# refresh-bio/vclust

Hardware: AMD Instinct MI355X
Metric: genome pairs/sec through prefilter+align (ani.tsv) (higher is better)
Workload: dtype u64

## Files before the change

vclust_amd/build.py:

```python
import os
import pathlib
import shutil
import subprocess
import sys

PKG_DIR = pathlib.Path(__file__).resolve().parent
ROOT = PKG_DIR.parent
CSRC = PKG_DIR / 'csrc'
LIB_PATH = PKG_DIR / 'libvclust_gpu.so'
ORACLE_DIR = ROOT / 'oracle'

SOURCES = ['vg_core.cpp', 'vg_genomes.cpp', 'vg_inflate.cpp', 'vg_io.cpp', 'vg_api.cpp', 'vg_synth.cpp', 'vg_prefilter.hip', 'vg_align.hip', 'vg_dist.hip', 'vg_cluster.hip', 'vg_dedup.hip']


def _hipcc() -> str:
    for cand in (os.environ.get('HIPCC'), shutil.which('hipcc'), '/opt/rocm/bin/hipcc'):
        if cand and pathlib.Path(cand).exists():
            return cand
    raise RuntimeError('hipcc not found (needs ROCm)')


def _stale(target: pathlib.Path, deps) -> bool:
    if not target.exists():
        return True
    t = target.stat().st_mtime
    return any(pathlib.Path(d).stat().st_mtime > t for d in deps)


def build_lib(force: bool = False, verbose: bool = False) -> pathlib.Path:
    srcs = [CSRC / s for s in SOURCES]
    deps = srcs + [CSRC / 'vg_common.h', CSRC / 'vg_window.h', ROOT / 'include' / 'vclust_gpu.h']
    if not force and not _stale(LIB_PATH, deps):
        return LIB_PATH
    obj_dir = PKG_DIR / '_obj'
    obj_dir.mkdir(exist_ok=True)
    hipcc = _hipcc()
    flags = ['--offload-arch=gfx950', '-O3', '-std=c++17', '-fPIC', '-Wall', '-Wno-unused-function',
             '-Wno-unused-result', f'-I{ROOT / "include"}']
    if os.environ.get('VG_LINES') == '1':
        flags.append('-gline-tables-only')
    if os.environ.get('VG_DEV') == '1':
        flags.append('-DVG_DEV_KERNELS')
    objs = []
    procs = []
    for s in srcs:
        o = obj_dir / (s.name + '.o')
        objs.append(o)
        if force or _stale(o, [s, CSRC / 'vg_common.h', CSRC / 'vg_window.h', ROOT / 'include' / 'vclust_gpu.h']):
            cmd = [hipcc, *flags, '-x', 'hip', '-c', str(s), '-o', str(o)]
            if verbose:
                print(' '.join(cmd), file=sys.stderr)
            procs.append((s, subprocess.Popen(cmd, stdout=subprocess.PIPE, stderr=subprocess.STDOUT, text=True)))
    for s, p in procs:
        out, _ = p.communicate()
        if p.returncode != 0:
            raise RuntimeError(f'hipcc failed on {s.name}:\n{out}')
        if verbose and out.strip():
            print(out, file=sys.stderr)
    cmd = [hipcc, '--offload-arch=gfx950', '-shared', '-fPIC', '-o', str(LIB_PATH), *map(str, objs), '-lz', '-lpthread', '-ldl']
    r = subprocess.run(cmd, stdout=subprocess.PIPE, stderr=subprocess.STDOUT, text=True)
    if r.returncode != 0:
        raise RuntimeError(f'link failed:\n{r.stdout}')
    return LIB_PATH


def build_oracle(verbose: bool = False) -> pathlib.Path:
    r = subprocess.run(['make', '-C', str(ORACLE_DIR)], stdout=subprocess.PIPE, stderr=subprocess.STDOUT, text=True)
    if r.returncode != 0:
        raise RuntimeError(f'oracle build failed:\n{r.stdout}')
    if verbose:
        print(r.stdout, file=sys.stderr)
    return ORACLE_DIR / '_build' / 'liboracle.so'


if __name__ == '__main__':
    force = '--force' in sys.argv
    print(build_lib(force=force, verbose=True))
    print(build_oracle(verbose=False))
```

vclust_amd/csrc/vg_align.hip:

```cpp
#include "vg_common.h"
#include "vg_window.h"
#include <rocprim/rocprim.hpp>
#include <algorithm>
#include <numeric>
#include <cstring>
#include <memory>
#include <mutex>
#include <optional>

namespace {

constexpr int RR_PAD = 128;

struct ref_desc {
    int64_t rr_w;
    int64_t mask_w;
    int64_t stab;
    int64_t sent;
    int32_t L;
    int32_t n_rr;
    int32_t genome;
    int32_t has_n;
    int32_t pos_bits;
    int32_t tag_bits;
// ... 371 lines not shown
#pragma unroll
                for (int u = 0; u < 4; ++u) {
                    const int p0 = pb + u * 4 * (int)blockDim.x;
                    if (p0 >= n4) continue;
                    const uint32_t sh = (uint32_t)(p0 & 31);
                    const uint32_t XL = __builtin_amdgcn_alignbit(w4[u].z, w4[u].x, sh), XH = __builtin_amdgcn_alignbit(w4[u].w, w4[u].y, sh);
                    const uint32_t XM = __builtin_amdgcn_alignbit(m1[u], m0[u], sh);
                    uint32_t out[4];
#pragma unroll
                    for (int j = 0; j < 4; ++j) {
                        const int p = p0 + j;
                        uint32_t bt = 0xffffffffu;
                        if (p + w <= rd.n_rr && ((XM >> j) & ((1u << w) - 1u)) == 0) {
                            const uint32_t xl = XL >> j, xh = XH >> j;
                            bt = bucket_of(xl, xh, msl) | (tag_of(xl, xh, msl, rd.tag_bits) << 18);
                            atomicAdd(&tab[(bt & 0x3ffffu) >> (big ? tsh : 0)], 1u);
                        }
                        out[j] = bt;
                    }
                    *reinterpret_cast<uint4*>(&scratch[p0]) = make_uint4(out[0], out[1], out[2], out[3]);
                }
            }
            __threadfence_block();
            __syncthreads();
            if (!big) {
                const uint32_t total = lds_scan_exclusive_waves(tab, n_cnt, part);
                const int nb = n_cnt;
                int w_lo = 0;
                while (w_lo < nb) {
                    const uint32_t base = tab[w_lo];
                    if (threadIdx.x == 0) s_whi = w_lo + 1;
                    lds_sync();
                    int best = w_lo + 1;
                    for (int b2 = w_lo + threadIdx.x; b2 < nb; b2 += blockDim.x) {
                        const uint32_t e2 = (b2 + 1 < nb) ? tab[b2 + 1] : total;
                        if (e2 - base <= (uint32_t)LDS_STAGE) best = b2 + 1; else break;
                    }
                    atomicMax(&s_whi, best);
                    lds_sync();
                    const int w_hi = s_whi;
                    const uint32_t e_lo = (w_lo + 1 < nb) ? tab[w_lo + 1] : total;
                    const bool direct = (e_lo - base > (uint32_t)LDS_STAGE);
                    lds_sync();
                    for (int pb = 4 * threadIdx.x; pb < n4; pb += 16 * blockDim.x) {
                        uint4 v[4];
#pragma unroll
                        for (int u = 0; u < 4; ++u) {
                            const int p0 = pb + u * 4 * (int)blockDim.x;
                            v[u] = (p0 < n4) ? *reinterpret_cast<const uint4*>(&scratch[p0]) : make_uint4(~0u, ~0u, ~0u, ~0u);
                        }
#pragma unroll
                        for (int u = 0; u < 4; ++u) {
                            const int p0 = pb + u * 4 * (int)blockDim.x;
                            const uint32_t bts[4] = { v[u].x, v[u].y, v[u].z, v[u].w };
#pragma unroll
                            for (int j = 0; j < 4; ++j) {
                                const uint32_t bt = bts[j];
                                const int b2 = (int)(bt & 0x3ffffu);
                                if (bt == 0xffffffffu || b2 < w_lo || b2 >= w_hi) continue;
                                const uint32_t ent = (uint32_t)(p0 + j) | ((bt >> 18) << rd.pos_bits);
                                const uint32_t slot = atomicAdd(&tab[b2], 1u);
                                if (direct) gent[slot] = ent; else stage[slot - base] = ent;
                            }
                        }
                    }
                    lds_sync();
                    if (!direct) {
                        const uint32_t cnt = tab[w_hi - 1] - base;
                        for (uint32_t i = threadIdx.x; i < cnt; i += blockDim.x) gent[base + i] = stage[i];
                    }
                    lds_sync();
                    w_lo = w_hi;
                }
                for (int i = threadIdx.x; i < nb; i += blockDim.x) gtab[i] = tab[i];
                lds_sync();
                continue;
            }
            const int n_bins = n_cnt;
            const uint32_t total = lds_scan_exclusive_waves(tab, n_bins, part);
            for (int i = threadIdx.x; i <= n_bins; i += blockDim.x) { s_bstart[i] = i < n_bins ? tab[i] : total; }
            lds_sync();
            for (int pb = 4 * threadIdx.x; pb < n4; pb += 16 * blockDim.x) {
                uint4 v[4];
#pragma unroll
                for (int u = 0; u < 4; ++u) {
                    const int p0 = pb + u * 4 * (int)blockDim.x;
                    v[u] = (p0 < n4) ? *reinterpret_cast<const uint4*>(&scratch[p0]) : make_uint4(~0u, ~0u, ~0u, ~0u);
                }
#pragma unroll
                for (int u = 0; u < 4; ++u) {
                    const int p0 = pb + u * 4 * (int)blockDim.x;
                    const uint32_t bts[4] = { v[u].x, v[u].y, v[u].z, v[u].w };
#pragma unroll
                    for (int j = 0; j < 4; ++j) {
                        if (bts[j] == 0xffffffffu) continue;
                        const uint32_t slot = atomicAdd(&tab[(bts[j] & 0x3ffffu) >> tsh], 1u);
                        binned[slot] = make_uint2(bts[j], (uint32_t)(p0 + j));
                    }
                }
            }
            __threadfence_block();
            __syncthreads();
            const int per_bin = 1 << tsh;
            int w_lo = 0;
            while (w_lo < n_bins) {
                if (threadIdx.x == 0) {
                    int hi = w_lo + 1;
                    while (hi < n_bins && s_bstart[hi + 1] - s_bstart[w_lo] <= (uint32_t)LDS_STAGE && (hi + 1 - w_lo) * per_bin <= LDS_TAB) ++hi;
                    s_whi = hi;
                }
                lds_sync();
                const int w_hi = s_whi;
                const uint32_t base = s_bstart[w_lo], cnt = s_bstart[w_hi] - base;
                const int nbw = (w_hi - w_lo) * per_bin; const uint32_t b_lo = (uint32_t)w_lo << tsh;
                const bool direct = cnt > (uint32_t)LDS_STAGE;
                for (int i = threadIdx.x; i < nbw; i += blockDim.x) tab[i] = 0;
                lds_sync();
                for (uint32_t i0 = threadIdx.x; i0 < cnt; i0 += 4 * blockDim.x) {
                    uint32_t bx[4];
#pragma unroll
                    for (int u = 0; u < 4; ++u) { const uint32_t i = i0 + u * blockDim.x; bx[u] = i < cnt ? binned[base + i].x : 0xffffffffu; }
#pragma unroll
                    for (int u = 0; u < 4; ++u) if (i0 + u * blockDim.x < cnt) atomicAdd(&tab[(bx[u] & 0x3ffffu) - b_lo], 1u);
                }
                lds_sync();
                lds_scan_exclusive_waves(tab, nbw, part);
                for (uint32_t i0 = threadIdx.x; i0 < cnt; i0 += 4 * blockDim.x) {
                    uint2 e4[4];
#pragma unroll
                    for (int u = 0; u < 4; ++u) { const uint32_t i = i0 + u * blockDim.x; e4[u] = i < cnt ? binned[base + i] : make_uint2(0u, 0u); }
#pragma unroll
                    for (int u = 0; u < 4; ++u) {
                        if (i0 + u * blockDim.x >= cnt) continue;
                        const uint2 e = e4[u];
                        const uint32_t ent = e.y | ((e.x >> 18) << rd.pos_bits);
                        const uint32_t slot = atomicAdd(&tab[(e.x & 0x3ffffu) - b_lo], 1u);
                        if (direct) gent[base + slot] = ent; else stage[slot] = ent;
                    }
                }
                lds_sync();
                if (!direct) for (uint32_t i = threadIdx.x; i < cnt; i += blockDim.x) gent[base + i] = stage[i];
                for (int i = threadIdx.x; i < nbw; i += blockDim.x) gtab[b_lo + i] = base + tab[i];
                lds_sync();
                w_lo = w_hi;
            }
        }
    }
}

constexpr int REG_IT = 24;
constexpr int REG_MAX_RR = 4 * 1024 * REG_IT - 256;
constexpr int REG_RR_WORDS = REG_MAX_RR / 16 + 32;
constexpr int REG_MK_WORDS = REG_MAX_RR / 32 + 16;
constexpr int REG_GEN_WORDS = 12288;
constexpr int REG_LDS_WORDS = LDS_TAB + REG_GEN_WORDS + REG_RR_WORDS + REG_MK_WORDS;
constexpr int REG_STAGE = REG_LDS_WORDS / 1024 * 1024;
constexpr int REG_STAGE0 = (REG_LDS_WORDS - LDS_TAB) / 1024 * 1024;
constexpr int REG_SLOT_BITS = 17;

template <int IT>
__device__ __forceinline__ void build_ref_reg(uint32_t* const lds, const ref_desc rd,
                  const uint32_t* __restrict__ gplanes, const uint32_t* __restrict__ nmask, const int64_t* __restrict__ base_off,
                  uint32_t* __restrict__ rr_pool, uint32_t* __restrict__ mask_pool, int msl,
                  uint32_t* __restrict__ stab_pool, uint32_t* __restrict__ sent_pool) {
    uint32_t* const tab = lds;
    uint32_t* const gw = lds + LDS_TAB;
    uint32_t* const gm = gw + 3328; uint32_t* const wtot = gw + 8192;
    uint32_t* const s_rr = gw + REG_GEN_WORDS;
    uint32_t* const s_mk = s_rr + REG_RR_WORDS;
    uint32_t* const stage = lds;
    const int nb = 1 << (2 * msl);
    {
        int tid = threadIdx.x;
        asm volatile("" : "+v"(tid));
        const int64_t g0 = base_off[rd.genome];
        const uint32_t* gpk = gplanes + (g0 >> 4); const uint32_t* gmk = nmask + (g0 >> 5);
        uint32_t* pk = rr_pool + rd.rr_w; uint32_t* mk = mask_pool + rd.mask_w;
        uint32_t* gtab = stab_pool + rd.stab; uint32_t* gent = sent_pool + rd.sent;
        const int n_gw = (rd.L >> 4) + 4, n_gm = (rd.L >> 5) + 3;
        for (int i = tid; i < n_gw; i += 1024) gw[i] = gpk[i];
        for (int i = tid; i < n_gm; i += 1024) gm[i] = gmk[i];
        for (int i = tid; i < nb; i += 1024) tab[i] = 0;
        lds_sync();
        const int chunks = (rd.n_rr + RR_PAD + 31) / 32 + 2;
        for (int ch = tid; ch < chunks; ch += 1024) {
            uint32_t lo, hi, m;
            rr_chunk_planes(gw, gm, rd.L, ch, &lo, &hi, &m);
            pk[2 * ch] = lo; pk[2 * ch + 1] = hi; mk[ch] = m;
            s_rr[2 * ch] = lo; s_rr[2 * ch + 1] = hi; s_mk[ch] = m;
        }
        lds_sync();
        uint32_t reg[IT][4];
        const int n4 = (rd.n_rr + 3) & ~3;
#pragma unroll
        for (int it = 0; it < IT; ++it) {
            const int p0 = 4 * (tid + 1024 * it);
            reg[it][0] = reg[it][1] = reg[it][2] = reg[it][3] = 0xffffffffu;
            if (p0 < n4) {
                const int wi = 2 * (p0 >> 5); const uint32_t sh = (uint32_t)(p0 & 31);
                const uint32_t XL = __builtin_amdgcn_alignbit(s_rr[wi + 2], s_rr[wi], sh), XH = __builtin_amdgcn_alignbit(s_rr[wi + 3], s_rr[wi + 1], sh);
                const uint32_t XM = __builtin_amdgcn_alignbit(s_mk[(p0 >> 5) + 1], s_mk[p0 >> 5], sh);
#pragma unroll
                for (int j = 0; j < 4; ++j) {
                    const int p = p0 + j;
                    if (p + msl <= rd.n_rr && ((XM >> j) & ((1u << msl) - 1u)) == 0) {
                        const uint32_t xl = XL >> j, xh = XH >> j;
                        const uint32_t bt = bucket_of(xl, xh, msl) | (tag_of(xl, xh, msl, rd.tag_bits) << 18);
                        atomicAdd(&tab[bt & 0x3ffffu], 1u);
                        reg[it][j] = bt;
                    }
                }
            }
            __builtin_amdgcn_sched_barrier(0);
        }
        lds_sync();
        const uint32_t total = lds_scan_exclusive_waves(tab, nb, wtot);
        uint32_t* const stage0 = lds + LDS_TAB;
        {
            uint32_t t4 = 4u * (uint32_t)tid;
            asm volatile("" : "+v"(t4));
#pragma unroll
            for (int it = 0; it < IT; ++it) {
#pragma unroll
                for (int j = 0; j < 4; ++j) {
                    const uint32_t bt = reg[it][j];
                    if (bt != 0xffffffffu) {
                        const uint32_t slot = atomicAdd(&tab[bt & 0x3ffffu], 1u);
                        reg[it][j] = slot | ((bt >> 18) << REG_SLOT_BITS);
                        if (slot < (uint32_t)REG_STAGE0) stage0[slot] = (t4 + (uint32_t)(4096 * it + j)) | ((bt >> 18) << rd.pos_bits);
                    }
                }
                __builtin_amdgcn_sched_barrier(0);
            }
        }
        lds_sync();
        auto copy_out = [&](uint32_t* dst, const uint32_t* src, uint32_t n) {
            for (uint32_t i = 4u * (uint32_t)tid; i < n; i += 4096u) {
                if (i + 4 <= n) { const uint4 v = make_uint4(src[i], src[i + 1], src[i + 2], src[i + 3]); __builtin_memcpy(dst + i, &v, 16); }
                else for (uint32_t j = i; j < n; ++j) dst[j] = src[j];
            }
        };
        copy_out(gtab, tab, (uint32_t)nb);
        copy_out(gent, stage0, min((uint32_t)REG_STAGE0, total));
        lds_sync();
        for (uint32_t base = REG_STAGE0; base < total; base += REG_STAGE) {
            uint32_t t4 = 4u * (uint32_t)tid;
            asm volatile("" : "+v"(t4));
#pragma unroll
            for (int it = 0; it < IT; ++it) {
#pragma unroll
                for (int j = 0; j < 4; ++j) {
                    uint32_t v = reg[it][j];
                    asm volatile("" : "+v"(v));
                    const uint32_t d = (v & ((1u << REG_SLOT_BITS) - 1u)) - base;
                    if (d < (uint32_t)REG_STAGE)
                        stage[d] = (t4 + (uint32_t)(4096 * it + j)) | ((v >> REG_SLOT_BITS) << rd.pos_bits);
                }
                __builtin_amdgcn_sched_barrier(0);
            }
            lds_sync();
            copy_out(gent + base, stage, min((uint32_t)REG_STAGE, total - base));
            lds_sync();
        }
    }
}
template <int IT>
__global__ void __launch_bounds__(1024)
k_build_index_reg(const ref_desc* __restrict__ refs, const int* __restrict__ slot_list, int n_list,
                  const uint32_t* __restrict__ gplanes, const uint32_t* __restrict__ nmask, const int64_t* __restrict__ base_off,
                  uint32_t* __restrict__ rr_pool, uint32_t* __restrict__ mask_pool, int msl,
                  uint32_t* __restrict__ stab_pool, uint32_t* __restrict__ sent_pool) {
    __shared__ uint32_t lds[REG_LDS_WORDS];
    for (int li = blockIdx.x; li < n_list; li += gridDim.x)
        build_ref_reg<IT>(lds, refs[slot_list[li]], gplanes, nmask, base_off, rr_pool, mask_pool, msl, stab_pool, sent_pool);
}

constexpr int MID_MAX_RR = 1 << 19;
constexpr int MID_STAGE = 23552;
__global__ void __launch_bounds__(1024)
k_build_index_mid(const ref_desc* __restrict__ refs, const int* __restrict__ slot_list, int n_list,
                  const uint32_t* __restrict__ gplanes, const uint32_t* __restrict__ nmask, const int64_t* __restrict__ base_off,
                  uint32_t* __restrict__ rr_pool, uint32_t* __restrict__ mask_pool, int msl,
                  uint32_t* __restrict__ stab_pool, uint32_t* __restrict__ sent_pool) {
    __shared__ uint32_t tab[LDS_TAB];
    __shared__ uint32_t stage[MID_STAGE];
    __shared__ uint32_t wtot[16];
    const int nb = 1 << (2 * msl);
    const int tid = threadIdx.x;
    for (int li = blockIdx.x; li < n_list; li += gridDim.x) {
        const ref_desc rd = refs[slot_list[li]];
        const int64_t g0 = base_off[rd.genome];
        const uint32_t* gpk = gplanes + (g0 >> 4); const uint32_t* gmk = nmask + (g0 >> 5);
        uint32_t* pk = rr_pool + rd.rr_w; uint32_t* mk = mask_pool + rd.mask_w;
        uint32_t* gtab = stab_pool + rd.stab; uint32_t* gent = sent_pool + rd.sent;
        const int chunks = (rd.n_rr + RR_PAD + 31) / 32 + 2;
        for (int ch = tid; ch < chunks; ch += 1024) {
            uint32_t lo, hi, m;
            rr_chunk_planes(gpk, gmk, rd.L, ch, &lo, &hi, &m);
            pk[2 * ch] = lo; pk[2 * ch + 1] = hi; mk[ch] = m;
        }
        for (int i = tid; i < nb; i += 1024) tab[i] = 0;
        __threadfence_block();
        __syncthreads();
        const int n16 = (rd.n_rr + 15) & ~15;
        auto load16 = [&](int p0, uint4& w, uint32_t& ok) {
            __builtin_memcpy(&w, pk + 2 * (p0 >> 5), 16);
            if (p0 & 16) { w.x = __builtin_amdgcn_alignbit(w.z, w.x, 16u); w.y = __builtin_amdgcn_alignbit(w.w, w.y, 16u); }
            const uint32_t m = __builtin_amdgcn_alignbit(mk[(p0 >> 5) + 1], mk[p0 >> 5], (uint32_t)(p0 & 31));
            uint32_t bad = m;
            for (int q = 1; q < msl; ++q) bad |= m >> q;
            ok = ~bad & 0xffffu;
            const int last = rd.n_rr - msl - p0;
            if (last < 15) ok &= last < 0 ? 0u : (2u << last) - 1u;
        };
        {
            int p0 = 16 * tid; uint4 w = make_uint4(0u, 0u, 0u, 0u); uint32_t ok = 0;
            if (p0 < n16) load16(p0, w, ok);
            while (p0 < n16) {
                const int pn = p0 + 16384; uint4 a = make_uint4(0u, 0u, 0u, 0u); uint32_t aok = 0;
                if (pn < n16) load16(pn, a, aok);
#pragma unroll
                for (int j = 0; j < 16; ++j)
                    if ((ok >> j) & 1u) atomicAdd(&tab[bucket_of(w.x >> j, w.y >> j, msl)], 1u);
                p0 = pn; w = a; ok = aok;
            }
        }
        lds_sync();
        const uint32_t total = lds_scan_exclusive_waves(tab, nb, wtot);
        for (int b_lo = 0; b_lo < nb;) {
            const uint32_t base = tab[b_lo];
            int lo = b_lo, hi = nb;
            while (lo < hi) { const int mid = (lo + hi + 1) >> 1; const uint32_t e = mid < nb ? tab[mid] : total; if (e - base <= (uint32_t)MID_STAGE) lo = mid; else hi = mid - 1; }
            const bool direct = lo == b_lo;
            const int gmask = (1 << msl) - 1;
            int b_hi = direct ? b_lo + 1 : lo;
            if (!direct) {
                if ((b_lo & gmask) == 0) { if ((b_hi & ~gmask) > b_lo) b_hi &= ~gmask; }
                else b_hi = min(b_hi, (b_lo | gmask) + 1);
            }
            const bool by_hi = ((b_lo | b_hi) & gmask) == 0;
            const uint32_t h_lo = (uint32_t)(b_lo >> msl), h_w = (uint32_t)((b_hi - b_lo) >> msl);
            const uint32_t w_end = b_hi < nb ? tab[b_hi] : total;
            const uint32_t width = (uint32_t)(b_hi - b_lo);
            lds_sync();
            if (w_end > base) {
                int p0 = 16 * tid; uint4 w = make_uint4(0u, 0u, 0u, 0u); uint32_t ok = 0;
                if (p0 < n16) load16(p0, w, ok);
                while (p0 < n16) {
                    const int pn = p0 + 16384; uint4 a = make_uint4(0u, 0u, 0u, 0u); uint32_t aok = 0;
                    if (pn < n16) load16(pn, a, aok);
                    uint32_t hits = 0;
                    if (by_hi) {
#pragma unroll
                        for (int j = 0; j < 16; ++j)
                            if (((w.y >> j) & (uint32_t)gmask) - h_lo < h_w) hits |= 1u << j;
                    } else {
#pragma unroll
                        for (int j = 0; j < 16; ++j)
                            if (bucket_of(w.x >> j, w.y >> j, msl) - (uint32_t)b_lo < width) hits |= 1u << j;
                    }
                    hits &= ok;
                    while (hits) {
                        const int j1 = __ffs(hits) - 1; hits &= hits - 1;
                        const int j2 = hits ? __ffs(hits) - 1 : -1; hits &= hits - 1;
                        const uint32_t xl1 = w.x >> j1, xh1 = w.y >> j1;
                        const uint32_t s1 = atomicAdd(&tab[bucket_of(xl1, xh1, msl)], 1u);
                        uint32_t xl2 = 0, xh2 = 0, s2 = 0;
                        if (j2 >= 0) {
                            xl2 = w.x >> j2; xh2 = w.y >> j2;
                            s2 = atomicAdd(&tab[bucket_of(xl2, xh2, msl)], 1u);
                        }
                        const uint32_t e1 = (uint32_t)(p0 + j1) | (tag_of(xl1, xh1, msl, rd.tag_bits) << rd.pos_bits);
                        if (direct) gent[s1] = e1; else stage[s1 - base] = e1;
                        if (j2 >= 0) {
                            const uint32_t e2 = (uint32_t)(p0 + j2) | (tag_of(xl2, xh2, msl, rd.tag_bits) << rd.pos_bits);
                            if (direct) gent[s2] = e2; else stage[s2 - base] = e2;
                        }
                    }
                    p0 = pn; w = a; ok = aok;
                }
                lds_sync();
                if (!direct) {
                    const uint32_t n = w_end - base;
                    for (uint32_t i = 4u * (uint32_t)tid; i < n; i += 4096u) {
                        if (i + 4 <= n && ((base + i) & 3u) == 0) { const uint4 v = make_uint4(stage[i], stage[i + 1], stage[i + 2], stage[i + 3]); __builtin_memcpy(gent + base + i, &v, 16); }
                        else for (uint32_t j = i; j < min(n, i + 4); ++j) gent[base + j] = stage[j];
                    }
                    lds_sync();
                }
            }
            b_lo = b_hi;
        }
        for (uint32_t i = 4u * (uint32_t)tid; i < (uint32_t)nb; i += 4096u) { const uint4 v = make_uint4(tab[i], tab[i + 1], tab[i + 2], tab[i + 3]); __builtin_memcpy(gtab + i, &v, 16); }
        lds_sync();
    }
}

__global__ void __launch_bounds__(256)
k_build_rr(const ref_desc* __restrict__ refs, const int* __restrict__ slot_list, int n_list,
           const int64_t* __restrict__ chunk_off ,
           const uint32_t* __restrict__ gplanes, const uint32_t* __restrict__ nmask, const int64_t* __restrict__ base_off,
           uint32_t* __restrict__ rr_pool, uint32_t* __restrict__ mask_pool) {
    const int64_t total = chunk_off[n_list];
    for (int64_t t = (int64_t)blockIdx.x * blockDim.x + threadIdx.x; t < total; t += (int64_t)gridDim.x * blockDim.x) {
        int lo = 0, hi = n_list - 1;
        while (lo < hi) { int mid = (lo + hi + 1) >> 1; if (chunk_off[mid] <= t) lo = mid; else hi = mid - 1; }
        const ref_desc rd = refs[slot_list[lo]];
        const int64_t ch = t - chunk_off[lo];
        const int64_t g0 = base_off[rd.genome];
        uint32_t pl_lo, pl_hi, m;
        rr_chunk_planes(gplanes + (g0 >> 4), nmask + (g0 >> 5), rd.L, ch, &pl_lo, &pl_hi, &m);
        rr_pool[rd.rr_w + 2 * ch] = pl_lo; rr_pool[rd.rr_w + 2 * ch + 1] = pl_hi;
        mask_pool[rd.mask_w + ch] = m;
    }
}

__global__ void __launch_bounds__(256)
k_index_pass(const ref_desc* __restrict__ refs, const int* __restrict__ slot_list, int n_list, const int64_t* __restrict__ chunk_off,
             const uint32_t* __restrict__ rr_pool, const uint32_t* __restrict__ mask_pool, int mal, int msl, int fill,
             uint32_t* __restrict__ stab_pool,
             uint32_t* __restrict__ sent_pool) {
    const int64_t total = chunk_off[n_list] * 32;
    (void)mal;
    for (int64_t t = (int64_t)blockIdx.x * blockDim.x + threadIdx.x; t < total; t += (int64_t)gridDim.x * blockDim.x) {
        int64_t chunk = t >> 5;
        int lo = 0, hi = n_list - 1;
        while (lo < hi) { int mid = (lo + hi + 1) >> 1; if (chunk_off[mid] <= chunk) lo = mid; else hi = mid - 1; }
        const ref_desc rd = refs[slot_list[lo]];
// ... 825 lines not shown
    VG_HIP(hipStreamSynchronize(s));
    VG_HIP(hipGetLastError());
    vg_host_mark("lz: kernels done");
    d_stats.download(stats, (size_t)n_tasks, s);
    VG_HIP(hipStreamSynchronize(s));
    vg_host_mark("lz: rows downloaded");
    if (want_regions) {
        for (int64_t t = 0; t < n_tasks && !first_pass.empty(); ++t)
            if (stats[t].n_regions != first_pass[(size_t)t].n_regions || stats[t].n_match != first_pass[(size_t)t].n_match || stats[t].aln_len != first_pass[(size_t)t].aln_len)
                throw vg_error(VG_EHIP, "internal error: the region pass and the counting pass of the LZ parse disagree on task " + std::to_string(t));
        vg_region* o = (vg_region*)malloc(sizeof(vg_region) * std::max<size_t>(1, h_regions.size()));
        if (!o) throw vg_error(VG_ENOMEM, "out of host memory");
        if (!h_regions.empty()) memcpy(o, h_regions.data(), sizeof(vg_region) * h_regions.size());
        *regions = o; if (n_regions) *n_regions = (int64_t)h_regions.size();
    }
    lz_keep_plan_host_side(plan);
    VG_API_END
}


namespace {
int64_t lz_ref_need(const vg_genomes* g, const vg_lz_params* p, uint32_t r, int64_t* chunks_out) {
    const int64_t stab_n = 1LL << (2 * p->msl);
    const int64_t n_rr = 2 * g->len[r] + 1;
    const int64_t chunks = (n_rr + RR_PAD + 31) / 32 + 2;
    if (chunks_out) *chunks_out = chunks;
    return chunks * 12 + (stab_n + n_rr) * 4;
}
int64_t lz_batch_budget(const vg_genomes* g, const vg_lz_params* p, const std::vector<uint32_t>& ref_ids) {
    int64_t batch_budget = g_index_budget_bytes;
    if (!g_index_budget_set && vg_one_shot()) {
        static const double gb = [] { const char* e = getenv("VG_ONESHOT_INDEX_GB"); const double v = e ? atof(e) : 0.0; return v >= 0.0625 ? v : 6.0; }();
        batch_budget = (int64_t)(gb * 1073741824.0);
    } else if (!g_index_budget_set) {
        int64_t all = 0;
        for (size_t ri = 0; ri < ref_ids.size() && all <= 2 * batch_budget; ++ri) all += lz_ref_need(g, p, ref_ids[ri], nullptr);
        if (all <= 2 * batch_budget) batch_budget = std::max(batch_budget, all);
    }
    return batch_budget;
}
void lz_plan_references(const vg_genomes* g, const vg_lz_params* p, lz_plan& P) {
    hipStream_t s = vg_stream();
    const std::vector<uint32_t>& ref_ids = P.ref_ids;
    const int64_t stab_n = 1LL << (2 * p->msl);
    P.mal = p->mal; P.msl = p->msl; P.g = g; P.n_genomes = g->n;
    const int64_t batch_budget = P.budget = lz_batch_budget(g, p, ref_ids);
    std::vector<lz_batch>& batches = P.batches;
    std::vector<ref_desc>& all_refs = P.all_refs;
    all_refs.assign(ref_ids.size(), ref_desc{});
    for (size_t ri = 0; ri < ref_ids.size();) {
        batches.emplace_back();
        lz_batch& B = batches.back();
        B.first_ref = (int)ri;
        int64_t bytes = 0;
        B.chunk_off.reserve(ref_ids.size() - ri + 1); B.reg_list.reserve(ref_ids.size() - ri);
        const int tag_want = 2 * (p->mal - p->msl);
        while (ri < ref_ids.size()) {
            const uint32_t r = ref_ids[ri];
            const int64_t L = g->len[r]; const int64_t n_rr = 2 * L + 1;
            int64_t chunks = 0; const int64_t need = lz_ref_need(g, p, r, &chunks);
            if (B.n_refs > 0 && bytes + need > batch_budget) break;
            ref_desc& rd = all_refs[ri];
            rd.rr_w = B.rr_words; rd.mask_w = B.mask_words; rd.stab = B.stab_tot; rd.sent = B.sent_n;
            rd.L = (int32_t)L; rd.n_rr = (int32_t)n_rr; rd.genome = (int32_t)r; rd.has_n = g->has_n[r];
            rd.pos_bits = n_rr <= 2 ? 1 : 64 - __builtin_clzll((unsigned long long)(n_rr - 1));
            rd.tag_bits = std::max(0, std::min({ tag_want, 14, 32 - rd.pos_bits }));
            B.rr_words += chunks * 2; B.mask_words += chunks; B.stab_tot += stab_n; B.sent_n += n_rr;
            B.chunk_off.push_back(B.chunk_off.back() + chunks);
            bytes += need; ++B.n_refs; ++ri;
        }
        const int n_refs = B.n_refs;
        for (int i = 0; i < n_refs; ++i) {
            const int gi = B.first_ref + i;
            const bool small = all_refs[(size_t)gi].n_rr <= (1 << 21) && p->msl <= 7;
            if (small && all_refs[(size_t)gi].n_rr <= REG_MAX_RR && !g_no_reg_build) B.reg_list.push_back(gi);
            else if (small && all_refs[(size_t)gi].n_rr <= MID_MAX_RR && !g_no_reg_build) B.mid_list.push_back(gi);
            else if (small) B.small_list.push_back(gi);
            else { B.large_list.push_back(gi); B.large_chunks.push_back(B.large_chunks.back() + (B.chunk_off[(size_t)i + 1] - B.chunk_off[(size_t)i])); }
        }
        auto longest_first = [&](std::vector<int>& list) {
            int32_t mn = INT32_MAX, mx = 0;
            for (int i : list) { mn = std::min(mn, all_refs[(size_t)i].n_rr); mx = std::max(mx, all_refs[(size_t)i].n_rr); }
            if (!list.empty() && (int64_t)mx * 4 > (int64_t)mn * 5 && (int64_t)(mx - mn) <= 8 * (int64_t)list.size() + 65536) {
                std::vector<int64_t> at((size_t)(mx - mn) + 2, 0);
                for (int i : list) at[(size_t)(mx - all_refs[(size_t)i].n_rr) + 1]++;
                for (size_t b = 1; b < at.size(); ++b) at[b] += at[b - 1];
                std::vector<int> sorted(list.size());
                for (int i : list) sorted[(size_t)at[(size_t)(mx - all_refs[(size_t)i].n_rr)]++] = i;
                list.swap(sorted);
            } else if (!list.empty() && (int64_t)mx * 4 > (int64_t)mn * 5) {
                std::vector<uint64_t> keyed(list.size());
                for (size_t i = 0; i < keyed.size(); ++i) keyed[i] = ((uint64_t)(0x7fffffffu - (uint32_t)all_refs[(size_t)list[i]].n_rr) << 32) | (uint32_t)list[i];
                std::sort(keyed.begin(), keyed.end());
                for (size_t i = 0; i < keyed.size(); ++i) list[i] = (int)(uint32_t)keyed[i];
            }
        };
        longest_first(B.reg_list); longest_first(B.mid_list); longest_first(B.small_list);
        {
            std::vector<int> by_class[6];
            for (int i : B.reg_list) {
                const int trips = (all_refs[(size_t)i].n_rr + 256 + 4095) / 4096;
                const int cls = trips > 20 ? 0 : trips > 16 ? 1 : trips > 12 ? 2 : trips > 8 ? 3 : trips > 4 ? 4 : 5;
                by_class[cls].push_back(i);
            }
            B.reg_list.clear();
            for (int c = 0; c < 6; ++c) { B.reg_list.insert(B.reg_list.end(), by_class[c].begin(), by_class[c].end()); B.reg_class_end[c] = (int)B.reg_list.size(); }
        }
        if (!B.small_list.empty()) {
            int64_t max_rr = 0; for (int i : B.small_list) max_rr = std::max<int64_t>(max_rr, all_refs[(size_t)i].n_rr);
            B.nblk_build = (int)std::min<size_t>(B.small_list.size(), 512);
            B.stride = (max_rr + 63) / 64 * 64;
            B.scratch_words = (int64_t)B.nblk_build * B.stride * 3;
        }
    }
    vg_host_mark("lz plan: batches cut");
    lz_plan_alloc(P);
}
void lz_plan_alloc(lz_plan& P) {
    hipStream_t s = vg_stream();
    std::vector<lz_batch>& batches = P.batches;
    std::vector<ref_desc>& all_refs = P.all_refs;
    P.d_refs.alloc(std::max<size_t>(1, all_refs.size()));
    if (!all_refs.empty()) P.d_refs.upload(all_refs.data(), all_refs.size(), s);
    vg_host_mark("lz plan: descriptors queued");
    size_t m_rr = 0, m_mask = 0, m_stab = 1, m_sent = 0, m_scr = 1, m_reg = 1, m_mid = 1, m_small = 1, m_large = 1, m_lch = 1;
    for (auto& B : batches) {
        m_rr = std::max(m_rr, (size_t)B.rr_words); m_mask = std::max(m_mask, (size_t)B.mask_words);
        m_stab = std::max(m_stab, (size_t)B.stab_tot); m_sent = std::max(m_sent, (size_t)B.sent_n); m_scr = std::max(m_scr, (size_t)B.scratch_words);
        m_reg = std::max(m_reg, B.reg_list.size()); m_mid = std::max(m_mid, B.mid_list.size()); m_small = std::max(m_small, B.small_list.size()); m_large = std::max(m_large, B.large_list.size());
        m_lch = std::max(m_lch, B.large_chunks.size());
    }
    lz_slot& L = P.slot;
    L.rr_pool.alloc(m_rr + 8); L.mask_pool.alloc(m_mask + 8); L.stab_pool.alloc(m_stab); L.sent_pool.alloc(m_sent + 4);
    L.scratch.alloc(m_scr); L.d_reg.alloc(m_reg); L.d_mid.alloc(m_mid); L.d_small.alloc(m_small); L.d_large.alloc(m_large); L.d_lchunk.alloc(m_lch);
}
void lz_build_batch(const vg_genomes* g, const vg_lz_params* p, lz_plan& P, size_t bi, hipStream_t sb) {
    lz_batch& B = P.batches[bi];
    lz_slot& L = P.slot;
    dbuf<ref_desc>& d_refs = P.d_refs;
    if (!B.reg_list.empty()) L.d_reg.upload(B.reg_list.data(), B.reg_list.size(), sb);
    if (!B.mid_list.empty()) L.d_mid.upload(B.mid_list.data(), B.mid_list.size(), sb);
    if (!B.small_list.empty()) L.d_small.upload(B.small_list.data(), B.small_list.size(), sb);
    if (!B.large_list.empty()) { L.d_large.upload(B.large_list.data(), B.large_list.size(), sb); L.d_lchunk.upload(B.large_chunks.data(), B.large_chunks.size(), sb); }
    const int64_t total_chunks = B.chunk_off.back();
    const uint32_t* gpl = vg_genome_planes(g, sb);
    vg_prof_scope ps("lz_build_index", (double)total_chunks * 32 * (0.375 + 0.375 + 4), sb);
    if (!B.large_list.empty()) VG_HIP(hipMemsetAsync(L.stab_pool.p, 0, (size_t)B.stab_tot * sizeof(uint32_t), sb));
    if (!B.reg_list.empty()) {
        auto launch = [&](auto kern, int first, int end) {
            if (end > first) hipLaunchKernelGGL(kern, dim3((unsigned)std::min(end - first, 512)), dim3(1024), 0, sb, d_refs.p, L.d_reg.p + first,
                                                end - first, gpl, g->d_nmask.p, g->d_base_off.p, L.rr_pool.p, L.mask_pool.p, p->msl, L.stab_pool.p, L.sent_pool.p);
        };
        const int* ce = B.reg_class_end;
        launch(k_build_index_reg<24>, 0, ce[0]); launch(k_build_index_reg<20>, ce[0], ce[1]); launch(k_build_index_reg<16>, ce[1], ce[2]);
        launch(k_build_index_reg<12>, ce[2], ce[3]); launch(k_build_index_reg<8>, ce[3], ce[4]); launch(k_build_index_reg<4>, ce[4], ce[5]);
    }
    if (!B.mid_list.empty()) {
        hipLaunchKernelGGL(k_build_index_mid, dim3((unsigned)std::min<size_t>(B.mid_list.size(), 512)), dim3(1024), 0, sb, d_refs.p, L.d_mid.p,
                           (int)B.mid_list.size(), gpl, g->d_nmask.p, g->d_base_off.p, L.rr_pool.p, L.mask_pool.p, p->msl,
                           L.stab_pool.p, L.sent_pool.p);
    }
    if (!B.small_list.empty()) {
        hipLaunchKernelGGL(k_build_index_lds, dim3(B.nblk_build), dim3(1024), 0, sb, d_refs.p, L.d_small.p, (int)B.small_list.size(),
                           gpl, g->d_nmask.p, g->d_base_off.p, L.rr_pool.p, L.mask_pool.p, p->mal, p->msl,
                           L.stab_pool.p, L.sent_pool.p, L.scratch.p, B.stride);
    }
    if (!B.large_list.empty()) {
        const int nl = (int)B.large_list.size(); const int64_t lc = B.large_chunks.back();
        hipLaunchKernelGGL(k_build_rr, dim3(grid_for(lc)), dim3(256), 0, sb, d_refs.p, L.d_large.p, nl, L.d_lchunk.p, gpl,
                           g->d_nmask.p, g->d_base_off.p, L.rr_pool.p, L.mask_pool.p);
        hipLaunchKernelGGL(k_index_pass, dim3(grid_for(lc * 32)), dim3(256), 0, sb, d_refs.p, L.d_large.p, nl, L.d_lchunk.p, L.rr_pool.p,
                           L.mask_pool.p, p->mal, p->msl, 0, L.stab_pool.p, L.sent_pool.p);
        hipLaunchKernelGGL(k_scan_tables, dim3(nl), dim3(256), 0, sb, d_refs.p, L.d_large.p, p->msl, L.stab_pool.p);
        hipLaunchKernelGGL(k_index_pass, dim3(grid_for(lc * 32)), dim3(256), 0, sb, d_refs.p, L.d_large.p, nl, L.d_lchunk.p, L.rr_pool.p,
                           L.mask_pool.p, p->mal, p->msl, 1, L.stab_pool.p, L.sent_pool.p);
    }
}
}

extern "C" int vg_lz_prepare(vg_genomes* g, const vg_pair_count* pairs, int64_t n_pairs, const vg_lz_params* p) {
    VG_API_BEGIN
    if (!g || (!pairs && n_pairs) || !p) throw vg_error(VG_EINVAL, "vg_lz_prepare: null argument");
    if (p->mal < 8 || p->mal > 31 || p->msl < 4 || p->msl > 12 || p->msl > p->mal) throw vg_error(VG_EINVAL, "mal must be 8..31, msl 4..12 and <= mal");
    vg_require_device();
    int rc = vg_genomes_to_device(g); if (rc) return rc;
    vg_lz_drop_prepared(nullptr);
    if (n_pairs == 0) return VG_OK;
    for (int i = 0; i < g->n; ++i) if (g->len[i] > (1 << 29)) throw vg_error(VG_EOVERFLOW, "genome longer than 2^29 bases");
    std::vector<uint8_t> is_ref((size_t)g->n, 0);
    for (int64_t i = 0; i < n_pairs; ++i) {
        if (pairs[i].a >= (uint32_t)g->n || pairs[i].b >= (uint32_t)g->n) throw vg_error(VG_EINVAL, "pair id out of range");
        is_ref[pairs[i].a] = 1; is_ref[pairs[i].b] = 1;
    }
    std::vector<uint32_t> ref_ids;
    for (int i = 0; i < g->n; ++i) if (is_ref[(size_t)i]) ref_ids.push_back((uint32_t)i);
    vg_host_mark("lz prepare: references listed");
    std::unique_ptr<lz_plan> plan;
    { std::lock_guard<std::mutex> lk(g_prep_mu); plan = lz_take_cached_plan(g, p, ref_ids); }
    if (plan) { lz_plan_alloc(*plan); vg_host_mark("lz prepare: plan of the last call taken over"); }
    else {
        plan.reset(new lz_plan);
        plan->ref_ids = std::move(ref_ids);
        plan->g = g;
        lz_plan_references(g, p, *plan);
        vg_host_mark("lz prepare: planned");
    }
    static const bool own_queue = [] { const char* e = vg_dev_getenv("VG_LZ_PREPARE_QUEUE"); return e && !strcmp(e, "own"); }();
    static const bool at_spgemm = [] { const char* e = vg_dev_getenv("VG_LZ_PREPARE_QUEUE"); return e && !strcmp(e, "spgemm"); }();
    if (at_spgemm) {
        lz_plan* raw = plan.get(); const vg_lz_params pp = *p;
        VG_HIP(hipEventCreateWithFlags(&plan->built_ev, hipEventDisableTiming));
        VG_HIP(hipEventRecord(plan->built_ev, vg_stream()));
        raw->batch0_built = false;
        vg_set_spgemm_hook([g, pp, raw] {
            static hipStream_t q = nullptr;
            if (!q && hipStreamCreateWithFlags(&q, hipStreamNonBlocking) != hipSuccess) return;
            hipEvent_t e0 = nullptr; if (hipEventCreateWithFlags(&e0, hipEventDisableTiming) != hipSuccess) return;
            (void)hipEventRecord(e0, vg_stream()); (void)hipStreamWaitEvent(q, e0, 0); (void)hipEventDestroy(e0);
            lz_build_batch(g, &pp, *raw, 0, q);
            (void)hipEventRecord(raw->built_ev, q);
            raw->batch0_built = true;
        });
        vg_host_mark("lz: first batch of indexes deferred to the SpGEMM");
        std::lock_guard<std::mutex> lk(g_prep_mu);
        g_prepared = std::move(plan);
        return VG_OK;
    }
    if (own_queue) {
        static hipStream_t q = nullptr;
        if (!q) VG_HIP(hipStreamCreateWithFlags(&q, hipStreamNonBlocking));
        hipEvent_t e0 = nullptr; VG_HIP(hipEventCreateWithFlags(&e0, hipEventDisableTiming));
        VG_HIP(hipEventRecord(e0, vg_stream())); VG_HIP(hipStreamWaitEvent(q, e0, 0)); (void)hipEventDestroy(e0);
        lz_build_batch(g, p, *plan, 0, q);
        VG_HIP(hipEventCreateWithFlags(&plan->built_ev, hipEventDisableTiming));
        VG_HIP(hipEventRecord(plan->built_ev, q));
    } else
    lz_build_batch(g, p, *plan, 0, vg_stream());
    plan->batch0_built = true;
    vg_host_mark("lz: first batch of indexes queued");
    std::lock_guard<std::mutex> lk(g_prep_mu);
    g_prepared = std::move(plan);
    VG_API_END
}

extern "C" void vg_set_index_budget(int64_t bytes) { if (bytes > (64 << 20)) { g_index_budget_bytes = bytes; g_index_budget_set = true; } }

namespace { __global__ void k_warm_align() {} }
void vg_warm_align(hipStream_t s) { hipLaunchKernelGGL(k_warm_align, dim3(1), dim3(64), 0, s); }
```

Baseline: 2.617 million.

## Prefetch next reference genome into registers during register-index build

Reorganizes the LDS layout of the register-class index build kernel, shrinking the genome staging region and placing RR planes beside the table. For IT<24 classes, each block now loads the next reference's genome planes into registers while histogramming the current one, then parks them in LDS, hiding global load latency across loop iterations. Also adds a compile-time-gated ablation kernel and timing harness for profiling build stages. Changes LDS size to a fixed 40960 words, which may affect occupancy and adds register pressure from the prefetch buffer.

```diff
diff --git a/vclust_amd/build.py b/vclust_amd/build.py
--- a/vclust_amd/build.py
+++ b/vclust_amd/build.py
@@ -41,6 +41,8 @@
         flags.append('-gline-tables-only')
     if os.environ.get('VG_DEV') == '1':
         flags.append('-DVG_DEV_KERNELS')
+    if os.environ.get('VG_BUILD_ABLATION') == '1':
+        flags.append('-DVG_BUILD_ABLATION')
     objs = []
     procs = []
     for s in srcs:
diff --git a/vclust_amd/csrc/vg_align.hip b/vclust_amd/csrc/vg_align.hip
--- a/vclust_amd/csrc/vg_align.hip
+++ b/vclust_amd/csrc/vg_align.hip
@@ -547,51 +547,74 @@
 constexpr int REG_MAX_RR = 4 * 1024 * REG_IT - 256;
 constexpr int REG_RR_WORDS = REG_MAX_RR / 16 + 32;
 constexpr int REG_MK_WORDS = REG_MAX_RR / 32 + 16;
-constexpr int REG_GEN_WORDS = 12288;
-constexpr int REG_LDS_WORDS = LDS_TAB + REG_GEN_WORDS + REG_RR_WORDS + REG_MK_WORDS;
-constexpr int REG_STAGE = REG_LDS_WORDS / 1024 * 1024;
-constexpr int REG_STAGE0 = (REG_LDS_WORDS - LDS_TAB) / 1024 * 1024;
+constexpr int REG_GW_WORDS = 3 * 1024;
+constexpr int REG_GM_WORDS = 2 * 1024;
+constexpr int REG_LDS_WORDS = 40960;
+constexpr int REG_WIN_WORDS = REG_LDS_WORDS - REG_GW_WORDS - REG_GM_WORDS;
+constexpr int REG_STAGE = REG_WIN_WORDS / 1024 * 1024;
+constexpr int REG_STAGE0 = (REG_WIN_WORDS - LDS_TAB) / 1024 * 1024;
+static_assert(LDS_TAB + REG_RR_WORDS + REG_MK_WORDS + 16 <= REG_WIN_WORDS, "RR planes and scan scratch beside the table");
+#define REG_PARKS_NEXT(IT) ((IT) < REG_IT)
+static_assert((REG_MAX_RR / 2 >> 4) + 4 <= REG_GW_WORDS && (REG_MAX_RR / 2 >> 5) + 3 <= REG_GM_WORDS, "genome corner");
+
+__device__ __forceinline__ void reg_genome_load(uint32_t (&v)[5], const ref_desc& nd, const uint32_t* __restrict__ gplanes,
+                                                const uint32_t* __restrict__ nmask, const int64_t* __restrict__ base_off, int tid) {
+    const int64_t g0 = base_off[nd.genome];
+    const uint32_t* gpk = gplanes + (g0 >> 4); const uint32_t* gmk = nmask + (g0 >> 5);
+    const int n_gw = (nd.L >> 4) + 4, n_gm = (nd.L >> 5) + 3;
+#pragma unroll
+    for (int k = 0; k < 3; ++k) { const int i = tid + 1024 * k; v[k] = i < n_gw ? gpk[i] : 0u; }
+#pragma unroll
+    for (int k = 0; k < 2; ++k) { const int i = tid + 1024 * k; v[3 + k] = i < n_gm ? gmk[i] : 0u; }
+}
+__device__ __forceinline__ void reg_genome_park(uint32_t* const lds, const uint32_t (&v)[5], int tid) {
+    uint32_t* const gw = lds + REG_WIN_WORDS; uint32_t* const gm = gw + REG_GW_WORDS;
+#pragma unroll
+    for (int k = 0; k < 3; ++k) gw[tid + 1024 * k] = v[k];
+#pragma unroll
+    for (int k = 0; k < 2; ++k) gm[tid + 1024 * k] = v[3 + k];
+}
 constexpr int REG_SLOT_BITS = 17;
 
 template <int IT>
-__device__ __forceinline__ void build_ref_reg(uint32_t* const lds, const ref_desc rd,
+__device__ __forceinline__ void build_ref_reg(uint32_t* const lds, const ref_desc rd, const ref_desc* __restrict__ refs, const int next,
                   const uint32_t* __restrict__ gplanes, const uint32_t* __restrict__ nmask, const int64_t* __restrict__ base_off,
                   uint32_t* __restrict__ rr_pool, uint32_t* __restrict__ mask_pool, int msl,
-                  uint32_t* __restrict__ stab_pool, uint32_t* __restrict__ sent_pool) {
+                  uint32_t* __restrict__ stab_pool, uint32_t* __restrict__ sent_pool, const int abl = 0) {
     uint32_t* const tab = lds;
-    uint32_t* const gw = lds + LDS_TAB;
-    uint32_t* const gm = gw + 3328; uint32_t* const wtot = gw + 8192;
-    uint32_t* const s_rr = gw + REG_GEN_WORDS;
+    uint32_t* const gw = lds + REG_WIN_WORDS;
+    uint32_t* const gm = gw + REG_GW_WORDS;
+    uint32_t* const s_rr = lds + LDS_TAB;
     uint32_t* const s_mk = s_rr + REG_RR_WORDS;
+    uint32_t* const wtot = s_mk + REG_MK_WORDS;
     uint32_t* const stage = lds;
     const int nb = 1 << (2 * msl);
     {
         int tid = threadIdx.x;
         asm volatile("" : "+v"(tid));
-        const int64_t g0 = base_off[rd.genome];
-        const uint32_t* gpk = gplanes + (g0 >> 4); const uint32_t* gmk = nmask + (g0 >> 5);
         uint32_t* pk = rr_pool + rd.rr_w; uint32_t* mk = mask_pool + rd.mask_w;
         uint32_t* gtab = stab_pool + rd.stab; uint32_t* gent = sent_pool + rd.sent;
-        const int n_gw = (rd.L >> 4) + 4, n_gm = (rd.L >> 5) + 3;
-        for (int i = tid; i < n_gw; i += 1024) gw[i] = gpk[i];
-        for (int i = tid; i < n_gm; i += 1024) gm[i] = gmk[i];
+        if (!REG_PARKS_NEXT(IT) && abl < 7) { uint32_t v[5]; reg_genome_load(v, rd, gplanes, nmask, base_off, tid); reg_genome_park(lds, v, tid); }
         for (int i = tid; i < nb; i += 1024) tab[i] = 0;
         lds_sync();
         const int chunks = (rd.n_rr + RR_PAD + 31) / 32 + 2;
-        for (int ch = tid; ch < chunks; ch += 1024) {
+        if (abl < 7) for (int ch = tid; ch < chunks; ch += 1024) {
             uint32_t lo, hi, m;
             rr_chunk_planes(gw, gm, rd.L, ch, &lo, &hi, &m);
             pk[2 * ch] = lo; pk[2 * ch + 1] = hi; mk[ch] = m;
             s_rr[2 * ch] = lo; s_rr[2 * ch + 1] = hi; s_mk[ch] = m;
         }
         lds_sync();
+        uint32_t nxt[5];
+        const bool has_next = REG_PARKS_NEXT(IT) && next >= 0 && abl < 7;
+        if (has_next) reg_genome_load(nxt, refs[next], gplanes, nmask, base_off, tid);
         uint32_t reg[IT][4];
         const int n4 = (rd.n_rr + 3) & ~3;
 #pragma unroll
         for (int it = 0; it < IT; ++it) {
             const int p0 = 4 * (tid + 1024 * it);
             reg[it][0] = reg[it][1] = reg[it][2] = reg[it][3] = 0xffffffffu;
-            if (p0 < n4) {
+            if (p0 < n4 && abl < 6) {
                 const int wi = 2 * (p0 >> 5); const uint32_t sh = (uint32_t)(p0 & 31);
                 const uint32_t XL = __builtin_amdgcn_alignbit(s_rr[wi + 2], s_rr[wi], sh), XH = __builtin_amdgcn_alignbit(s_rr[wi + 3], s_rr[wi + 1], sh);
                 const uint32_t XM = __builtin_amdgcn_alignbit(s_mk[(p0 >> 5) + 1], s_mk[p0 >> 5], sh);
@@ -601,17 +624,18 @@
                     if (p + msl <= rd.n_rr && ((XM >> j) & ((1u << msl) - 1u)) == 0) {
                         const uint32_t xl = XL >> j, xh = XH >> j;
                         const uint32_t bt = bucket_of(xl, xh, msl) | (tag_of(xl, xh, msl, rd.tag_bits) << 18);
-                        atomicAdd(&tab[bt & 0x3ffffu], 1u);
+                        if (abl < 5) atomicAdd(&tab[bt & 0x3ffffu], 1u);
                         reg[it][j] = bt;
                     }
                 }
             }
             __builtin_amdgcn_sched_barrier(0);
         }
+        if (has_next) reg_genome_park(lds, nxt, tid);
         lds_sync();
         const uint32_t total = lds_scan_exclusive_waves(tab, nb, wtot);
         uint32_t* const stage0 = lds + LDS_TAB;
-        {
+        if (abl < 4) {
             uint32_t t4 = 4u * (uint32_t)tid;
             asm volatile("" : "+v"(t4));
 #pragma unroll
@@ -622,7 +646,7 @@
                     if (bt != 0xffffffffu) {
                         const uint32_t slot = atomicAdd(&tab[bt & 0x3ffffu], 1u);
                         reg[it][j] = slot | ((bt >> 18) << REG_SLOT_BITS);
-                        if (slot < (uint32_t)REG_STAGE0) stage0[slot] = (t4 + (uint32_t)(4096 * it + j)) | ((bt >> 18) << rd.pos_bits);
+                        if (slot < (uint32_t)REG_STAGE0 && abl < 2) stage0[slot] = (t4 + (uint32_t)(4096 * it + j)) | ((bt >> 18) << rd.pos_bits);
                     }
                 }
                 __builtin_amdgcn_sched_barrier(0);
@@ -635,10 +659,10 @@
                 else for (uint32_t j = i; j < n; ++j) dst[j] = src[j];
             }
         };
-        copy_out(gtab, tab, (uint32_t)nb);
-        copy_out(gent, stage0, min((uint32_t)REG_STAGE0, total));
+        if (abl < 3) copy_out(gtab, tab, (uint32_t)nb);
+        if (abl < 1) copy_out(gent, stage0, min((uint32_t)REG_STAGE0, total));
         lds_sync();
-        for (uint32_t base = REG_STAGE0; base < total; base += REG_STAGE) {
+        for (uint32_t base = REG_STAGE0; base < total && abl < 2; base += REG_STAGE) {
             uint32_t t4 = 4u * (uint32_t)tid;
             asm volatile("" : "+v"(t4));
 #pragma unroll
@@ -654,7 +678,7 @@
                 __builtin_amdgcn_sched_barrier(0);
             }
             lds_sync();
-            copy_out(gent + base, stage, min((uint32_t)REG_STAGE, total - base));
+            if (abl < 1) copy_out(gent + base, stage, min((uint32_t)REG_STAGE, total - base));
             lds_sync();
         }
     }
@@ -666,9 +690,39 @@
                   uint32_t* __restrict__ rr_pool, uint32_t* __restrict__ mask_pool, int msl,
                   uint32_t* __restrict__ stab_pool, uint32_t* __restrict__ sent_pool) {
     __shared__ uint32_t lds[REG_LDS_WORDS];
-    for (int li = blockIdx.x; li < n_list; li += gridDim.x)
-        build_ref_reg<IT>(lds, refs[slot_list[li]], gplanes, nmask, base_off, rr_pool, mask_pool, msl, stab_pool, sent_pool);
-}
+    if ((int)blockIdx.x >= n_list) return;
+    if (REG_PARKS_NEXT(IT)) {
+        uint32_t v[5];
+        reg_genome_load(v, refs[slot_list[blockIdx.x]], gplanes, nmask, base_off, (int)threadIdx.x);
+        reg_genome_park(lds, v, (int)threadIdx.x);
+    }
+    for (int li = blockIdx.x; li < n_list; li += gridDim.x) {
+        const int nx = li + (int)gridDim.x;
+        build_ref_reg<IT>(lds, refs[slot_list[li]], refs, nx < n_list ? slot_list[nx] : -1, gplanes, nmask, base_off, rr_pool, mask_pool, msl,
+                          stab_pool, sent_pool);
+    }
+}
+#ifdef VG_BUILD_ABLATION
+template <int IT>
+__global__ void __launch_bounds__(1024)
+k_build_index_reg_abl(const ref_desc* __restrict__ refs, const int* __restrict__ slot_list, int n_list,
+                      const uint32_t* __restrict__ gplanes, const uint32_t* __restrict__ nmask, const int64_t* __restrict__ base_off,
+                      uint32_t* __restrict__ rr_pool, uint32_t* __restrict__ mask_pool, int msl,
+                      uint32_t* __restrict__ stab_pool, uint32_t* __restrict__ sent_pool, int abl) {
+    __shared__ uint32_t lds[REG_LDS_WORDS];
+    if ((int)blockIdx.x >= n_list) return;
+    if (REG_PARKS_NEXT(IT)) {
+        uint32_t v[5];
+        reg_genome_load(v, refs[slot_list[blockIdx.x]], gplanes, nmask, base_off, (int)threadIdx.x);
+        reg_genome_park(lds, v, (int)threadIdx.x);
+    }
+    for (int li = blockIdx.x; li < n_list; li += gridDim.x) {
+        const int nx = li + (int)gridDim.x;
+        build_ref_reg<IT>(lds, refs[slot_list[li]], refs, nx < n_list ? slot_list[nx] : -1, gplanes, nmask, base_off, rr_pool, mask_pool, msl,
+                          stab_pool, sent_pool, abl);
+    }
+}
+#endif
 
 constexpr int MID_MAX_RR = 1 << 19;
 constexpr int MID_STAGE = 23552;
@@ -1800,6 +1854,26 @@
                                                 end - first, gpl, g->d_nmask.p, g->d_base_off.p, L.rr_pool.p, L.mask_pool.p, p->msl, L.stab_pool.p, L.sent_pool.p);
         };
         const int* ce = B.reg_class_end;
+#ifdef VG_BUILD_ABLATION
+        static const bool ablate = [] { const char* e = vg_dev_getenv("VG_BUILD_ABLATE"); return e && *e == '1'; }();
+        if (ablate && ce[1] > ce[0]) {
+            hipEvent_t e0, e1; VG_HIP(hipEventCreate(&e0)); VG_HIP(hipEventCreate(&e1));
+            fprintf(stderr, "build ablation, %d references of class 20:", ce[1] - ce[0]);
+            for (int a = 0; a <= 7; ++a) {
+                float best = 1e30f;
+                for (int r = 0; r < 3; ++r) {
+                    VG_HIP(hipEventRecord(e0, sb));
+                    hipLaunchKernelGGL(k_build_index_reg_abl<20>, dim3((unsigned)std::min(ce[1] - ce[0], 512)), dim3(1024), 0, sb, d_refs.p, L.d_reg.p + ce[0],
+                                       ce[1] - ce[0], gpl, g->d_nmask.p, g->d_base_off.p, L.rr_pool.p, L.mask_pool.p, p->msl, L.stab_pool.p, L.sent_pool.p, a);
+                    VG_HIP(hipEventRecord(e1, sb)); VG_HIP(hipEventSynchronize(e1));
+                    float ms = 0; VG_HIP(hipEventElapsedTime(&ms, e0, e1)); best = std::min(best, ms);
+                }
+                fprintf(stderr, " abl%d=%.3f", a, best);
+            }
+            fprintf(stderr, "\n");
+            VG_HIP(hipEventDestroy(e0)); VG_HIP(hipEventDestroy(e1));
+        }
+#endif
         launch(k_build_index_reg<24>, 0, ce[0]); launch(k_build_index_reg<20>, ce[0], ce[1]); launch(k_build_index_reg<16>, ce[1], ce[2]);
         launch(k_build_index_reg<12>, ce[2], ce[3]); launch(k_build_index_reg<8>, ce[3], ce[4]); launch(k_build_index_reg<4>, ce[4], ce[5]);
     }
```

After: 2.638 million (median of 6 runs). Within noise of the previous version (+0.8%).
